# MoHawastaken/Gaussian-Process-Regression

Hardware: AMD Instinct MI355X
Metric: GPR predict-step achieved fp64 TFLOP/s (kernel fill + Cholesky + solves + mean/variance), n x n sqexp (higher is better)
Workload: dtype f64; 1 GPU; c4: n=65536 d=8 sqrexp GPR fit+predict, n*=65536 (reference test-grid rule), noise=0.1; n=65536, d=8, n_star=65536, kernel=sqrexp, parallelism=1-D block-cyclic 512-column panels over 1 GPU(s), test points sliced

## Files before the change

gaussian-process-regression_amd/_native.py:

```python
from __future__ import annotations

import ctypes as C
import os
import threading

import numpy as np

_HERE = os.path.dirname(os.path.abspath(__file__))
LIB_PATH = os.path.join(_HERE, "lib", "libgprc_native" + os.environ.get("GPRC_LIB_SUFFIX", "") + ".so")

CONSTANT, LINEAR, POLYNOMIAL, SQREXP, GAMMAEXP, RATQUAD, SQREXP_ARD = range(7)

OK = 0
GPC_REFERENCE_STOP = 1
ERR_ARG, ERR_HIP, ERR_NOMEM, ERR_NOT_PD, ERR_DIVERGED, ERR_MAXITER, ERR_NO_DEVICE = -1, -2, -3, -4, -5, -6, -7


class GprcError(RuntimeError):

    def __init__(self, status: int, message: str):
        super().__init__(f"gprc native error {status}: {message}")
        self.status = status
        self.message = message

# ... 83 lines not shown
    "gprc_mgpu_gpr_get_noise": (C.c_int, [_vp, C.POINTER(C.c_double)]),
    "gprc_mgpu_model_rank": (C.c_int, [_vp, C.c_int, C.POINTER(_vp)]),
    "gprc_mgpu_model_free": (C.c_int, [_vp]),
    "gprc_mvn_factor": (C.c_int, [_vp, _vp, _i64, _i64, C.c_double, _vp, C.POINTER(C.c_int)]),
    "gprc_mvn_sample": (C.c_int, [_vp, _vp, _i64, _i64, _vp, C.c_double, _vp, _i64, _vp, C.POINTER(C.c_int)]),
    "gprc_sym_eigen": (C.c_int, [_vp, _vp, _i64, _i64, _vp, _vp, C.POINTER(C.c_int)]),
    "gprc_combine_all": (C.c_int, [_vp, _vp, C.POINTER(_i64), C.c_int, _vp]),
    "gprc_prof_enable": (C.c_int, [C.c_int]),
    "gprc_prof_panel_trace": (C.c_int, [_vp, C.c_int, C.POINTER(_i64), C.c_int]),
    "gprc_prof_service_trace": (C.c_int, [_vp, C.POINTER(_i64), C.c_int]),
    "gprc_prof_wait_timeout": (C.c_int, [C.POINTER(C.c_int), C.c_int]),
    "gprc_prof_reset": (C.c_int, []),
    "gprc_prof_kinds": (C.c_int, []),
    "gprc_prof_summary": (C.c_int, [C.c_int, C.POINTER(_i64), C.POINTER(C.c_double), C.POINTER(C.c_double), C.POINTER(C.c_double)]),
    "gprc_dev_solve_rows": (C.c_int, [_vp, _vp, _vp, _i64, _vp, _i64, _i64]),
    "gprc_dev_reverse_factor": (C.c_int, [_vp, _vp, _vp, _i64, _vp, _vp]),
}

_lib = None
_lib_lock = threading.Lock()


def _share_hip_runtime_with_torch() -> None:
    import importlib.util
    import sys
    if "torch" in sys.modules:
        return
    try:
        spec = importlib.util.find_spec("torch")
    except (ImportError, ValueError):
# ... 120 lines not shown
```

gaussian-process-regression_amd/csrc/chol_tile.h:

```cpp
#pragma once
#include <utility>

#include "gprc_internal.h"

namespace gprc {

typedef double double4_t __attribute__((ext_vector_type(4)));

namespace {

constexpr int PB = 128;

constexpr int BLD = 144;
constexpr int PB_SMEM_DOUBLES = PB * BLD + 512 + PB;
constexpr size_t PB_SMEM_BYTES = PB_SMEM_DOUBLES * sizeof(double);

__device__ __forceinline__ void sqrt_rsqrt(double d, double& root, double& rinv) {
  double r = __builtin_amdgcn_rsq(d);
#pragma unroll
  for (int it = 0; it < 2; ++it) {
    const double e = fma(-(d * r), r, 1.0);
    r = fma(0.5 * r, e, r);
  }
  double l = d * r;
// ... 185 lines not shown
        const int c = ty + TYS * (k0 + k);
        if (i >= c) A[i + (int64_t)c * lda] = lv[k];
        winv[i + c * PB] = wv[k];
      }
    }
  }
  POTF2_STAMP(19);
}

constexpr int G_KB = 16;
constexpr int G_LDT = 144;
constexpr int G_BUF = G_KB * G_LDT;
constexpr int G_SMEM_DOUBLES = 4 * G_BUF;
constexpr size_t G_SMEM_BYTES = G_SMEM_DOUBLES * sizeof(double);

__device__ __forceinline__ void read_ops(const double* Ac, const double* Bc, int kk, double (&a)[4], double (&b)[4]) {
#pragma unroll
  for (int m = 0; m < 4; ++m) a[m] = Ac[kk * 4 * G_LDT + m * 16];
#pragma unroll
  for (int n = 0; n < 4; ++n) b[n] = Bc[kk * 4 * G_LDT + n * 16];
}
template <int NEG>
__device__ __forceinline__ void mma_step(const double (&a)[4], const double (&b)[4], double4_t (&acc)[4][4]) {
#pragma unroll
  for (int m = 0; m < 4; ++m)
#pragma unroll
    for (int n = 0; n < 4; ++n) acc[m][n] = __builtin_amdgcn_mfma_f64_16x16x4f64(b[n], a[m], acc[m][n], 0, 0, NEG);
}

typedef __attribute__((address_space(1))) const void* gptr_t;
typedef __attribute__((address_space(3))) void* lptr_t;
__device__ __forceinline__ void dma_ktile(const double* Ag, int64_t lda, const double* Bg, int64_t ldb, double* Asb, double* Bsb) {
#pragma unroll
  for (int i = 0; i < 4; ++i) {
    __builtin_amdgcn_global_load_lds((gptr_t)(Ag + (int64_t)(4 * i) * lda), (lptr_t)(Asb + 4 * i * G_LDT), 16, 0, 0);
// ... 13 lines not shown
  }
}

template <bool SEG>
__device__ __forceinline__ const char* strip_ktile_s(const double* B, int64_t ldb, int64_t brow, int kt, int wave, int64_t& ld) {
  if constexpr (SEG) {
    const int pp = kt / (NB / 16);
    ld = panel_ld(ldb, pp);
    return reinterpret_cast<const char*>(B + panel_offset(ldb, pp) + (brow - (int64_t)pp * NB) + (int64_t)((kt % (NB / 16)) * 16 + wave) * ld);
  } else {
    ld = ldb;
    return reinterpret_cast<const char*>(B + (int64_t)(kt * 16 + wave) * ldb);
  }
}

template <bool SET, bool SEG = false, bool SEGA = false, bool SSQ = false, bool LDSOUT = false, bool ILV = true, int CORE = 2, bool WT = false>
__device__ __forceinline__ void gemm_tile_128(double* C, int64_t ldc, const double* A, int64_t lda, const double* B,
                                              int64_t ldb, int K, double* smem, int64_t brow = 0, int64_t arow = 0, int kt0 = 0,
                                              double* ssq = nullptr, int tid = -1, double* lds_out = nullptr) {
  const int t = tid < 0 ? (int)threadIdx.x : tid, lane = t & 63;
  const int wave = __builtin_amdgcn_readfirstlane(t >> 6);
  const int wr = wave >> 1, wc = wave & 1;
  const int fk = lane >> 4, fr = lane & 15;
  double* As = smem;
  double* Bs = smem + 2 * G_BUF;

  constexpr int NEG = SET ? 0 : 1;
  double* Cw = C + (wr * 64 + fr) + (int64_t)(wc * 64 + fk) * ldc;
  double4_t acc[4][4];
#pragma unroll
  for (int n = 0; n < 4; ++n)
#pragma unroll
    for (int r = 0; r < 4; ++r)
#pragma unroll
      for (int m = 0; m < 4; ++m) acc[m][n][r] = SET ? 0.0 : Cw[m * 16 + (int64_t)(n * 16 + 4 * r) * ldc];

  int64_t ldak, ldbk;
  const double* Ag = strip_ktile<SEGA>(A, lda, arow, SEGA ? kt0 : 0, lane, wave, ldak);
  const double* Bg = strip_ktile<SEG>(B, ldb, brow, SEG ? kt0 : 0, lane, wave, ldbk);
  const int srow = wave * G_LDT;
  const int foff = fr + fk * G_LDT;

  constexpr int LGKM0 = 0xC07F;
  const int KT = K / G_KB;
  dma_ktile(Ag, ldak, Bg, ldbk, As + srow, Bs + srow);
  __builtin_amdgcn_s_waitcnt(0x0F70);
  __syncthreads();
  if (KT > 1) {
    Ag = strip_ktile<SEGA>(A, lda, arow, (SEGA ? kt0 : 0) + 1, lane, wave, ldak);
    Bg = strip_ktile<SEG>(B, ldb, brow, (SEG ? kt0 : 0) + 1, lane, wave, ldbk);
    dma_ktile(Ag, ldak, Bg, ldbk, As + G_BUF + srow, Bs + G_BUF + srow);
  }
  if constexpr (!SEGA) Ag = A + 2 * lane + (int64_t)(2 * G_KB + wave) * lda;
  if constexpr (!SEG) Bg = B + 2 * lane + (int64_t)(2 * G_KB + wave) * ldb;
  double a0[4], b0[4], a1[4], b1[4], a2[4], b2[4], a3[4], b3[4];
  read_ops(As + wr * 64 + foff, Bs + wc * 64 + foff, 0, a0, b0);
  read_ops(As + wr * 64 + foff, Bs + wc * 64 + foff, 1, a1, b1);
  if constexpr (ILV && CORE == 2) {
  const unsigned lane_off = 16u * (unsigned)lane;
  const unsigned ldsA = (unsigned)(uintptr_t)(lptr_t)(As + srow), ldsB = (unsigned)(uintptr_t)(lptr_t)(Bs + srow);
  const unsigned aBase = (unsigned)(uintptr_t)(lptr_t)(As + wr * 64 + foff), bBase = (unsigned)(uintptr_t)(lptr_t)(Bs + wc * 64 + foff);
  int64_t ldas, ldbs;
  const char* Asg = strip_ktile_s<SEGA>(A, lda, arow, (SEGA ? kt0 : 0) + 2, wave, ldas);
  const char* Bsg = strip_ktile_s<SEG>(B, ldb, brow, (SEG ? kt0 : 0) + 2, wave, ldbs);
#define GPRC_SB __builtin_amdgcn_sched_barrier(0);
#define GPRC_M(A_, B_, i) acc[(i) >> 2][(i) & 3] = __builtin_amdgcn_mfma_f64_16x16x4f64(B_[(i) & 3], A_[(i) >> 2], acc[(i) >> 2][(i) & 3], 0, 0, NEG); GPRC_SB
#define GPRC_RD(dst, base, off) asm volatile("ds_read_b64 %0, %1 offset:%2" : "=v"(dst) : "v"(base), "n"(off));
#define GPRC_RA(buf, kk, r, A_) GPRC_RD(A_[2 * (r)], aBase, ((buf) * G_BUF + (kk) * 4 * G_LDT + (2 * (r)) * 16) * 8) GPRC_RD(A_[2 * (r) + 1], aBase, ((buf) * G_BUF + (kk) * 4 * G_LDT + (2 * (r) + 1) * 16) * 8) GPRC_SB
#define GPRC_RB(buf, kk, r, B_) GPRC_RD(B_[2 * (r)], bBase, ((buf) * G_BUF + (kk) * 4 * G_LDT + (2 * (r)) * 16) * 8) GPRC_RD(B_[2 * (r) + 1], bBase, ((buf) * G_BUF + (kk) * 4 * G_LDT + (2 * (r) + 1) * 16) * 8) GPRC_SB
#define GPRC_READY(cnt, A_, B_) asm volatile("s_waitcnt lgkmcnt(" #cnt ")" : "+v"(A_[0]), "+v"(A_[1]), "+v"(A_[2]), "+v"(A_[3]), "+v"(B_[0]), "+v"(B_[1]), "+v"(B_[2]), "+v"(B_[3])); GPRC_SB
#define GPRC_BLOCK_R(A_, B_, buf, kk, RA_, RB_, cond)                                                               \
  GPRC_M(A_, B_, 0) GPRC_M(A_, B_, 1) if (cond) { GPRC_RA(buf, kk, 0, RA_) }                                        \
  GPRC_M(A_, B_, 2) GPRC_M(A_, B_, 3) if (cond) { GPRC_RA(buf, kk, 1, RA_) }                                        \
  GPRC_M(A_, B_, 4) GPRC_M(A_, B_, 5) if (cond) { GPRC_RB(buf, kk, 0, RB_) }                                        \
  GPRC_M(A_, B_, 6) GPRC_M(A_, B_, 7) if (cond) { GPRC_RB(buf, kk, 1, RB_) }                                        \
  GPRC_M(A_, B_, 8) GPRC_M(A_, B_, 9) GPRC_M(A_, B_, 10) GPRC_M(A_, B_, 11) GPRC_M(A_, B_, 12) GPRC_M(A_, B_, 13) GPRC_M(A_, B_, 14) GPRC_M(A_, B_, 15)
#define GPRC_DMA(i, buf, more2)                                                                                      \
  if (more2) {                                                                                                      \
    if ((i) < 4) asm volatile("s_mov_b32 m0, %2\n\ts_nop 0\n\tglobal_load_lds_dwordx4 %0, %1" :: "v"(lane_off), "s"(Asg + (int64_t)(4 * (i)) * ldas * 8), "s"(ldsA + (unsigned)(((buf) * G_BUF + 4 * (i) * G_LDT) * 8)) : "memory"); \
    else asm volatile("s_mov_b32 m0, %2\n\ts_nop 0\n\tglobal_load_lds_dwordx4 %0, %1" :: "v"(lane_off), "s"(Bsg + (int64_t)(4 * ((i) - 4)) * ldbs * 8), "s"(ldsB + (unsigned)(((buf) * G_BUF + 4 * ((i) - 4) * G_LDT) * 8)) : "memory"); \
    GPRC_SB                                                                                                         \
  }
#define GPRC_KTILE(buf, more1, more2)                                                                                \
  {                                                                                                                 \
    GPRC_SB                                                                                                         \
    GPRC_READY(8, a0, b0)                                                                                           \
    GPRC_BLOCK_R(a0, b0, buf, 2, a2, b2, true)                                                                      \
    GPRC_READY(8, a1, b1)                                                                                           \
    GPRC_BLOCK_R(a1, b1, buf, 3, a3, b3, true)                                                                      \
    GPRC_READY(8, a2, b2)                                                                                           \
    GPRC_M(a2, b2, 0) GPRC_M(a2, b2, 1) GPRC_M(a2, b2, 2) GPRC_M(a2, b2, 3)                                         \
    if (more1) {                                                                                                    \
       \
                           \
      asm volatile("s_waitcnt vmcnt(0) lgkmcnt(0)" ::: "memory");                                                   \
      __builtin_amdgcn_s_barrier();                                                                                 \
      GPRC_SB                                                                                                       \
    }                                                                                                               \
    GPRC_M(a2, b2, 4) if (more1) { GPRC_RA(1 - (buf), 0, 0, a0) }                                                   \
// ... 42 lines not shown
  GPRC_M(A_, B_, 0) GPRC_M(A_, B_, 1) if (cond) { GPRC_RA(Ap_, kk, 0, RA_) }                                        \
  GPRC_M(A_, B_, 2) GPRC_M(A_, B_, 3) if (cond) { GPRC_RA(Ap_, kk, 1, RA_) }                                        \
  GPRC_M(A_, B_, 4) GPRC_M(A_, B_, 5) if (cond) { GPRC_RB(Bp_, kk, 0, RB_) }                                        \
  GPRC_M(A_, B_, 6) GPRC_M(A_, B_, 7) if (cond) { GPRC_RB(Bp_, kk, 1, RB_) }                                        \
  GPRC_M(A_, B_, 8) GPRC_M(A_, B_, 9) GPRC_M(A_, B_, 10) GPRC_M(A_, B_, 11) GPRC_M(A_, B_, 12) GPRC_M(A_, B_, 13) GPRC_M(A_, B_, 14) GPRC_M(A_, B_, 15)
#define GPRC_DMA(i, more2)                                                                                           \
  if (more2) {                                                                                                      \
    if ((i) < 4) __builtin_amdgcn_global_load_lds((gptr_t)(Ag + (int64_t)(4 * (i)) * ldak), (lptr_t)(As + cur + srow + 4 * (i) * G_LDT), 16, 0, 0); \
    else __builtin_amdgcn_global_load_lds((gptr_t)(Bg + (int64_t)(4 * ((i) - 4)) * ldbk), (lptr_t)(Bs + cur + srow + 4 * ((i) - 4) * G_LDT), 16, 0, 0); \
    GPRC_SB                                                                                                         \
  }
#define GPRC_KTILE(more1, more2)                                                                                     \
  {                                                                                                                 \
    const int cur = (kt & 1) * G_BUF, nxt = G_BUF - cur;                                                            \
    const double* Ac = As + cur + wr * 64 + foff;                                                                   \
    const double* Bc = Bs + cur + wc * 64 + foff;                                                                   \
    const double* An = As + nxt + wr * 64 + foff;                                                                   \
    const double* Bn = Bs + nxt + wc * 64 + foff;                                                                   \
    GPRC_SB                                                                                                         \
    GPRC_BLOCK_R(a0, b0, Ac, Bc, 2, a2, b2, true)                                                                   \
    GPRC_BLOCK_R(a1, b1, Ac, Bc, 3, a3, b3, true)                                                                   \
    GPRC_M(a2, b2, 0) GPRC_M(a2, b2, 1) GPRC_M(a2, b2, 2) GPRC_M(a2, b2, 3)                                         \
    if (more1) {                                                                                                    \
       \
                         \
      asm volatile("s_waitcnt vmcnt(0) lgkmcnt(0)" ::: "memory");                                                   \
      __builtin_amdgcn_s_barrier();                                                                                 \
      GPRC_SB                                                                                                       \
      if (more2) {                                                                                                  \
        if constexpr (SEGA || SEG) {                                                                                \
          const bool boundary = ((kt0 + kt + 2) % (NB / 16)) == 0;                                                  \
          if constexpr (SEGA) { if (boundary) Ag = strip_ktile<true>(A, lda, arow, kt0 + kt + 2, lane, wave, ldak); else Ag += (int64_t)G_KB * ldak; } \
          if constexpr (SEG) { if (boundary) Bg = strip_ktile<true>(B, ldb, brow, kt0 + kt + 2, lane, wave, ldbk); else Bg += (int64_t)G_KB * ldbk; } \
// ... 20 lines not shown
      const bool more1 = kt + 1 < KT;
      GPRC_KTILE(more1, false)
    }
  }
#undef GPRC_KTILE
#undef GPRC_DMA
#undef GPRC_BLOCK_R
#undef GPRC_RA
#undef GPRC_RB
#undef GPRC_M
#undef GPRC_SB
  } else {
  for (int kt = 0; kt < KT; ++kt) {
    const int cur = (kt & 1) * G_BUF, nxt = G_BUF - cur;
    const double* Ac = As + cur + wr * 64 + foff;
    const double* Bc = Bs + cur + wc * 64 + foff;
    const double* An = As + nxt + wr * 64 + foff;
    const double* Bn = Bs + nxt + wc * 64 + foff;
    __builtin_amdgcn_s_waitcnt(LGKM0);
    read_ops(Ac, Bc, 2, a2, b2);
    mma_step<NEG>(a0, b0, acc);
    __builtin_amdgcn_sched_barrier(0);
    __builtin_amdgcn_s_waitcnt(LGKM0);
    read_ops(Ac, Bc, 3, a3, b3);
    mma_step<NEG>(a1, b1, acc);
    __builtin_amdgcn_sched_barrier(0);
    __builtin_amdgcn_s_waitcnt(LGKM0);
    if (kt + 1 < KT) {
      asm volatile("s_waitcnt vmcnt(0)" ::: "memory");
      __syncthreads();
      if (kt + 2 < KT) {
        if constexpr (SEGA || SEG) {
          const bool boundary = ((kt0 + kt + 2) % (NB / 16)) == 0;
// ... 10 lines not shown
    __builtin_amdgcn_sched_barrier(0);
    __builtin_amdgcn_s_waitcnt(LGKM0);
    if (kt + 1 < KT) read_ops(An, Bn, 1, a1, b1);
    mma_step<NEG>(a3, b3, acc);
    __builtin_amdgcn_sched_barrier(0);
  }

  }

#pragma unroll
  for (int n = 0; n < 4; ++n)
#pragma unroll
    for (int r = 0; r < 4; ++r)
#pragma unroll
      for (int m = 0; m < 4; ++m) {
        if constexpr (WT) __hip_atomic_store(&Cw[m * 16 + (int64_t)(n * 16 + 4 * r) * ldc], acc[m][n][r], __ATOMIC_RELAXED, __HIP_MEMORY_SCOPE_AGENT);
        else Cw[m * 16 + (int64_t)(n * 16 + 4 * r) * ldc] = acc[m][n][r];
      }

  if constexpr (LDSOUT) {
    __syncthreads();
    constexpr int LDO = 144;
#pragma unroll
    for (int n = 0; n < 4; ++n)
#pragma unroll
      for (int r = 0; r < 4; ++r)
#pragma unroll
        for (int m = 0; m < 4; ++m) {
          const int row = wr * 64 + fr + m * 16, col = wc * 64 + fk + n * 16 + 4 * r;
          lds_out[row + col * LDO] = (row >= col) ? acc[m][n][r] : 0.0;
        }
  }

  if constexpr (SSQ) {
    double rs[4];
#pragma unroll
    for (int m = 0; m < 4; ++m) {
      double q = 0.0;
#pragma unroll
      for (int n = 0; n < 4; ++n)
#pragma unroll
        for (int r = 0; r < 4; ++r) q = fma(acc[m][n][r], acc[m][n][r], q);
      q += __shfl_xor(q, 16, 64);
      q += __shfl_xor(q, 32, 64);
      rs[m] = q;
    }
    __syncthreads();
    if (fk == 0) {
#pragma unroll
// ... 47 lines not shown
```

gaussian-process-regression_amd/csrc/gprc_internal.h:

```cpp
#pragma once
#include <hip/hip_runtime.h>
#include <stdint.h>
#include <atomic>
#include <string>

#include "../../include/gprc_native.h"

namespace gprc {

#ifndef GPRC_NB
#define GPRC_NB 512
#endif
constexpr int NB = GPRC_NB;
constexpr int NBI = 128;
constexpr int TPP = NB / NBI;
constexpr int MAX_PARAMS = 256;
constexpr int MAX_DEVICES = 64;
static_assert(NB % NBI == 0 && NB >= NBI, "panel width must be a multiple of the 128 block");

__host__ __device__ static inline int64_t pad_up(int64_t n, int64_t m) { return (n + m - 1) / m * m; }
__host__ __device__ static inline int64_t panel_offset(int64_t n_pad, int64_t p) { return (int64_t)NB * (p * n_pad - (int64_t)NB * p * (p - 1) / 2); }
__host__ __device__ static inline int64_t panel_ld(int64_t n_pad, int64_t p) { return n_pad - p * NB; }
template <typename T>
__host__ __device__ constexpr T panel_tiles(T P, T q) { return TPP * TPP * (P - q) - TPP * (TPP - 1) / 2; }
constexpr int SERVICE_CORE_WGS = 3 + TPP + TPP * (TPP + 1) / 2;
constexpr int CHAIN_HELPERS = 4;

void set_error(const std::string& msg);
int hip_fail(hipError_t e, const char* what, const char* file, int line);

#define GPRC_HIP(call)                                                          \
  do {                                                                          \
    hipError_t e__ = (call);                                                    \
    if (e__ != hipSuccess) return ::gprc::hip_fail(e__, #call, __FILE__, __LINE__); \
  } while (0)
#define GPRC_TRY(call)          \
  do {                          \
    int rc__ = (call);          \
    if (rc__ != 0) return rc__; \
  } while (0)
#define GPRC_LAUNCH_CHECK() GPRC_HIP(hipGetLastError())
// ... 55 lines not shown

int64_t grad_partial_rows();
int launch_grad_contract(hipStream_t s, const KernelSpec& ks, const double* X, int64_t d, int64_t n, const double* alpha, const double* W,
                         int64_t ld, double* part);
int launch_gpc_grad_contract(hipStream_t s, const KernelSpec& ks, const double* X, int64_t d, int64_t n, const double* a, const double* sw,
                             const double* u, const double* g, const double* W, int64_t ld, double* part);

int64_t pred_grad_stripes(int64_t n_pad);
int launch_pred_grad(hipStream_t s, const KernelSpec& ks, const double* Xs, int64_t m, int64_t m_pad, const double* X, int64_t n, int64_t n_pad,
                     int64_t d, const double* alpha, const double* W, int64_t ldw, double* pmean, double* pvar);
int launch_pred_grad_sum(hipStream_t s, const KernelSpec& ks, const double* part, int64_t n_pad, int64_t d, int64_t m_pad, int64_t m, bool variance,
                         double* out);

int launch_solve_panel_fused(hipStream_t s, double* vt, int64_t ldv, int64_t m_pad, const double* packed, int64_t n_pad, int64_t p,
                             const double* winv, double* sspart, int64_t ss_stride = 0);
int launch_trsm_panel(hipStream_t s, double* X, int64_t ldx, int64_t M, const double* winv, double* ssq = nullptr);
int launch_gemm_nt(hipStream_t s, double* C, int64_t ldc, const double* A, int64_t lda, const double* B, int64_t ldb,
                   int64_t M, int64_t N, int64_t K, int lower, int kind);
int launch_solve_left(hipStream_t s, double* vt, int64_t ldv, int64_t m_pad, const double* packed, int64_t n_pad, int64_t j, int64_t G,
                      int64_t tri_row0 = -1);
int launch_trailing_update(hipStream_t s, double* packed, int64_t n_pad, int64_t p, int64_t q_begin, int64_t q_end,
                           int64_t q_stride);
int launch_trailing_range(hipStream_t s, double* packed, int64_t n_pad, int64_t p_begin, int64_t p_end, int64_t q_begin, int64_t q_end,
                          int64_t q_stride);

int launch_potf2_inv(hipStream_t s, double* A, int64_t lda, double* winv, int* info_dev, int col0);
int launch_panel_fused(hipStream_t s, double* packed, int64_t n_pad, int64_t p, double* winv, int* info_dev, void* sync16, int trace);
size_t panel_service_sync_bytes(int64_t P);
int launch_panel_service(hipStream_t s, double* packed, int64_t n_pad, double* winv, int* info_dev, void* sync, void* trace, double* inv,
                         int64_t p_begin, int64_t p_end, bool split, int part);
// ... 41 lines not shown
```

gaussian-process-regression_amd/csrc/gprc_sched.hip:

```cpp
#include <algorithm>
#include <cstdlib>
#include <cstring>

#include "gprc_host.h"

namespace gprc {

static bool panel_steps() {
  static const bool steps = [] { const char* e = std::getenv("GPRC_PANEL"); return e && std::strcmp(e, "steps") == 0; }();
  return steps;
}

int factor_subpanel(gprc_ctx* ctx, double* packed, int64_t n_pad, int64_t p, int j, int part, double* winv, int* info_dev) {
  if (part == 2) return 0;
  hipStream_t s = ctx->stream;
  const int64_t ld = panel_ld(n_pad, p);
  double* pan = packed + panel_offset(n_pad, p);
  const int64_t cj = (int64_t)j * NBI;
  double* wblk = winv + (p * (NB / NBI) + j) * NBI * NBI;
  if (cj > 0)
    GPRC_TRY(launch_gemm_nt(s, pan + cj + cj * ld, ld, pan + cj, ld, pan + cj, ld, ld - cj, NBI, cj, 1, PK_GEMM_INNER));
  GPRC_TRY(launch_potf2_inv(s, pan + cj + cj * ld, ld, wblk, info_dev, (int)(p * NB + cj)));
  const int64_t below = ld - cj - NBI;
  if (below > 0) GPRC_TRY(launch_trsm_panel(s, pan + (cj + NBI) + cj * ld, ld, below, wblk));
// ... 148 lines not shown
              "under a tool that serialises dispatches (e.g. rocprofv3 --pmc) set GPRC_SERVICE=0");
    return GPRC_ERR_HIP;
  }
  return 0;
}

int solve_rows(gprc_ctx* ctx, const double* packed, const double* winv, int64_t n_pad, double* vt, int64_t ldv, int64_t m_pad,
               double* sspart, int64_t tri_row0, int64_t p_end) {
  hipStream_t s = ctx->stream;
  const int64_t P = p_end >= 0 ? std::min(p_end, n_pad / NB) : n_pad / NB;
  const char* mode = std::getenv("GPRC_SOLVE");
  int64_t G = (4096 + (m_pad / 128) * (NB / NBI) - 1) / ((m_pad / 128) * (NB / NBI));
  if (mode && std::strcmp(mode, "left") == 0) G = 1;
  else if (mode && std::atoi(mode) > 0) G = std::atoi(mode);
  if ((mode && std::strcmp(mode, "right") == 0) || G > P) G = P;
  auto rows_of = [&](int64_t col_end) {
    if (tri_row0 < 0) return m_pad;
    return std::max<int64_t>(0, std::min<int64_t>(m_pad, pad_up(col_end - tri_row0, 128)));
  };
  for (int64_t g0 = 0; g0 < P; g0 += G) {
    const int64_t g1 = std::min(P, g0 + G);
    const int64_t mg = rows_of(g1 * NB);
    if (mg == 0) continue;
    GPRC_TRY(launch_solve_left(s, vt, ldv, mg, packed, n_pad, g0, g1 - g0, tri_row0));
    static const bool solve_panel_steps = [] { const char* e = std::getenv("GPRC_SOLVE_PANEL"); return e && std::strcmp(e, "steps") == 0; }();
    for (int64_t p = g0; p < g1; ++p) {
      const int64_t ld = panel_ld(n_pad, p);
      const double* pan = packed + panel_offset(n_pad, p);
      const int64_t mp = rows_of((p + 1) * NB);
      if (mp == 0) continue;
      if (!solve_panel_steps) {
        GPRC_TRY(launch_solve_panel_fused(s, vt, ldv, mp, packed, n_pad, p, winv, sspart, m_pad));
      } else
      for (int j = 0; j < NB / NBI; ++j) {
        const int64_t cj = p * NB + (int64_t)j * NBI;
        const double* wblk = winv + (p * (NB / NBI) + j) * NBI * NBI;
        if (j > 0)
          GPRC_TRY(launch_gemm_nt(s, vt + cj * ldv, ldv, vt + p * NB * ldv, ldv, pan + (int64_t)j * NBI, ld, mp, NBI, (int64_t)j * NBI, 0,
                                  PK_GEMM_INNER));
        GPRC_TRY(launch_trsm_panel(s, vt + cj * ldv, ldv, mp, wblk, sspart ? sspart + (cj / NBI) * m_pad : nullptr));
// ... 69 lines not shown
  return factor_all_async(ctx, packed, n_pad, winv, info_dev, inv);
}
int gprc_factor_service(int on) {
  const int was = g_service_off.load() ? 0 : 1;
  if (on == 0) g_service_off.store(true);
  else if (on > 0) g_service_off.store(false);
  return was;
}

int gprc_dev_solve_rows(gprc_ctx* ctx, const double* packed, const double* winv, int64_t n_pad, double* vt,
                        int64_t ld, int64_t m_pad) {
  GPRC_TRY(use_device_unless(ctx, m_pad % 128 || n_pad % NB || ld < m_pad || ld % 2, "solve_rows: bad padding"));
  return solve_rows(ctx, packed, winv, n_pad, vt, ld, m_pad);
}

int gprc_dev_reverse_factor(gprc_ctx* ctx, const double* packed, const double* winv, int64_t n_pad, double* packed_rev, double* winv_rev) {
  GPRC_TRY(use_device_unless(ctx, !packed || !winv || !packed_rev || !winv_rev || n_pad <= 0 || n_pad % NB, "dev_reverse_factor: bad arguments"));
  return launch_reverse_factor(ctx->stream, packed, winv, n_pad, packed_rev, winv_rev);
}

int gprc_prof_panel_trace(gprc_ctx* ctx, int side, int64_t* ticks_out, int n) {
  GPRC_TRY(use_device_unless(ctx, !ticks_out || n < 1 || n > 24, "prof_panel_trace: 1..24 stamps"));
  GPRC_HIP(hipDeviceSynchronize());
  GPRC_HIP(hipMemcpy(ticks_out, static_cast<char*>(ctx->sync_dev) + (side ? 256 : 0) + 64, sizeof(int64_t) * (size_t)n, hipMemcpyDeviceToHost));
  return 0;
}

int gprc_prof_service_trace(gprc_ctx* ctx, int64_t* ticks_out, int panels) {
  GPRC_TRY(use_device_unless(ctx, !ticks_out || panels < 1 || panels > SVC_TRACE_PANELS, "prof_service_trace: 1..48 panels"));
  if (!ctx->svc_trace) { set_error("prof_service_trace: no traced sweep on this context (set GPRC_SERVICE_TRACE before the first call)"); return GPRC_ERR_ARG; }
// ... 76 lines not shown
```

gaussian-process-regression_amd/csrc/kernels_gemm.hip:

```cpp
#include <algorithm>

#include "chol_tile.h"

namespace gprc {
namespace {

template <int ROLE>
__global__ __launch_bounds__(256, 2) void gemm_nt_kernel(double* C, int64_t ldc, const double* A, int64_t lda,
                                                         const double* B, int64_t ldb, int tiles_m, int tiles_n, int K,
                                                         int lower, int group) {
  extern __shared__ __attribute__((aligned(16))) double smem[];
  const unsigned ntiles = (unsigned)tiles_m * (unsigned)tiles_n;
  for (unsigned t = blockIdx.x; t < ntiles; t += gridDim.x) {
    const unsigned id = ROLE == PK_INV_GEMM ? t : xcd_remap(t, ntiles);
    int tr, tc;
    group_tile(id, tiles_m, tiles_n, group, tr, tc);
    if (lower && tc > tr) continue;
    const int64_t k0 = ROLE == PK_INV_GEMM ? (int64_t)tr * 128 : 0;
    gemm_tile_128<false>(C + (int64_t)tr * 128 + (int64_t)tc * 128 * ldc, ldc, A + (int64_t)tr * 128 + k0 * lda, lda,
                         B + (int64_t)tc * 128 + k0 * ldb, ldb, K - (int)k0, smem);
    __syncthreads();
  }
}

// ... 47 lines not shown
__global__ __launch_bounds__(256, 2) void solve_panel_fused_kernel(double* vt, int64_t ldv, const double* packed, int64_t n_pad, int p,
                                                                   const double* winv, double* sspart, int64_t m_pad) {
  extern __shared__ __attribute__((aligned(16))) double smem[];
  const int64_t ld = panel_ld(n_pad, p);
  const double* pan = packed + panel_offset(n_pad, p);
  double* strip = vt + (int64_t)blockIdx.x * 128 + (int64_t)p * NB * ldv;
  for (int j = 0; j < TPP; ++j) {
    double* C = strip + (int64_t)j * NBI * ldv;
    if (j > 0) {
      gemm_tile_128<false>(C, ldv, strip, ldv, pan + (int64_t)j * NBI, ld, j * NBI, smem);
      asm volatile("s_waitcnt vmcnt(0)" ::: "memory");
      __syncthreads();
    }
    const double* wblk = winv + ((int64_t)p * TPP + j) * NBI * NBI;
    double* ssq = SSQ ? sspart + ((int64_t)p * TPP + j) * m_pad + (int64_t)blockIdx.x * 128 : nullptr;
    gemm_tile_128<true, false, false, SSQ>(C, ldv, C, ldv, wblk, 128, 128, smem, 0, 0, 0, ssq);
    asm volatile("s_waitcnt vmcnt(0)" ::: "memory");
    __syncthreads();
  }
}

__global__ __launch_bounds__(256, 2) void trailing_range_kernel(double* packed, int64_t n_pad, int p_begin, int p_end, int q_begin,
                                                                int q_stride, int n_targets, int ntiles) {
  extern __shared__ __attribute__((aligned(16))) double smem[];
  const int P = (int)(n_pad / NB);
  int id = (int)xcd_remap(blockIdx.x, (unsigned)ntiles);
  int q, tr, tc;
  if (!target_tile(id, P, q_begin, q_stride, n_targets, q)) return;
  panel_tile(id, tr, tc);
  const int64_t ldq = panel_ld(n_pad, q);
  double* Cq = packed + panel_offset(n_pad, q);
  const int64_t row = (int64_t)q * NB + (int64_t)tr * 128, col = (int64_t)q * NB + (int64_t)tc * 128;
  gemm_tile_128<false, true, true>(Cq + (int64_t)tr * 128 + (int64_t)tc * 128 * ldq, ldq, packed, n_pad, packed, n_pad,
                                   (p_end - p_begin) * NB, smem, col, row, p_begin * (NB / 16));
}

}

int launch_solve_left(hipStream_t s, double* vt, int64_t ldv, int64_t m_pad, const double* packed, int64_t n_pad, int64_t j, int64_t G,
                      int64_t tri_row0) {
  if (j <= 0 || m_pad <= 0 || G <= 0) return 0;
  if (m_pad % 128) { set_error("solve_left: m_pad must be a multiple of 128"); return GPRC_ERR_ARG; }
  if ((j + G) * NB > n_pad) { set_error("solve_left: panel group beyond the factor"); return GPRC_ERR_ARG; }
  GPRC_TRY(ensure_dynamic_lds<solve_left_kernel>(G_SMEM_BYTES));
  const int64_t N = G * NB, tiles = (m_pad / 128) * (N / 128), K = j * NB;
  double fl = 2.0 * (double)m_pad * N * (double)K;
  if (tri_row0 >= 0) {
    fl = 0.0;
    for (int64_t tr = 0; tr < m_pad / 128; ++tr) fl += 2.0 * 128.0 * N * (double)std::max<int64_t>(0, K - std::max<int64_t>(0, tri_row0 + tr * 128));
  }
  ProfScope ps(s, PK_SOLVE_LEFT, fl, 8.0 * (2.0 * m_pad * N + (double)m_pad * K + (double)N * K));
  hipLaunchKernelGGL(solve_left_kernel, dim3((unsigned)tiles), dim3(256), G_SMEM_BYTES, s, vt, ldv, packed, n_pad,
                     (int)j, (int)(m_pad / 128), (int)(N / 128), 8, tri_row0);
  GPRC_LAUNCH_CHECK();
  return 0;
}

int launch_solve_panel_fused(hipStream_t s, double* vt, int64_t ldv, int64_t m_pad, const double* packed, int64_t n_pad, int64_t p,
                             const double* winv, double* sspart, int64_t ss_stride) {
  if (m_pad <= 0) return 0;
  if (ss_stride <= 0) ss_stride = m_pad;
  if (m_pad % 128) { set_error("solve_panel_fused: m_pad must be a multiple of 128"); return GPRC_ERR_ARG; }
  GPRC_TRY(sspart ? ensure_dynamic_lds<solve_panel_fused_kernel<true>>(G_SMEM_BYTES) : ensure_dynamic_lds<solve_panel_fused_kernel<false>>(G_SMEM_BYTES));
  const double M = (double)m_pad;
  ProfScope ps(s, PK_SOLVE_PANEL, M * 128.0 * 128.0 * TPP + 2.0 * M * 128.0 * 128.0 * (TPP * (TPP - 1) / 2), 8.0 * 2.0 * M * NB);
  if (sspart) hipLaunchKernelGGL(solve_panel_fused_kernel<true>, dim3((unsigned)(m_pad / 128)), dim3(256), G_SMEM_BYTES, s, vt, ldv, packed, n_pad, (int)p, winv, sspart, ss_stride);
  else hipLaunchKernelGGL(solve_panel_fused_kernel<false>, dim3((unsigned)(m_pad / 128)), dim3(256), G_SMEM_BYTES, s, vt, ldv, packed, n_pad, (int)p, winv, sspart, ss_stride);
  GPRC_LAUNCH_CHECK();
  return 0;
}

int launch_trsm_panel(hipStream_t s, double* X, int64_t ldx, int64_t M, const double* winv, double* ssq) {
  if (M <= 0) return 0;
  if (M % 128) { set_error("trsm_panel: M must be a multiple of 128"); return GPRC_ERR_ARG; }
  GPRC_TRY(ssq ? ensure_dynamic_lds<trsm_panel_kernel<true>>(G_SMEM_BYTES) : ensure_dynamic_lds<trsm_panel_kernel<false>>(G_SMEM_BYTES));
  ProfScope ps(s, PK_TRSM_PANEL, 1.0 * M * 128 * 128, 8.0 * 2 * M * 128);
  if (ssq) hipLaunchKernelGGL(trsm_panel_kernel<true>, dim3((unsigned)(M / 128)), dim3(256), G_SMEM_BYTES, s, X, ldx, winv, ssq);
  else hipLaunchKernelGGL(trsm_panel_kernel<false>, dim3((unsigned)(M / 128)), dim3(256), G_SMEM_BYTES, s, X, ldx, winv, ssq);
  GPRC_LAUNCH_CHECK();
  return 0;
}

// ... 63 lines not shown
```

include/gprc_native.h:

```cpp
#ifndef GPRC_NATIVE_H
#define GPRC_NATIVE_H

#include <stdint.h>

#ifdef __cplusplus
extern "C" {
#endif

#define GPRC_ABI_VERSION 1

#if defined(__GNUC__)
#define GPRC_API __attribute__((visibility("default")))
#else
#define GPRC_API
#endif

typedef enum {
  GPRC_CONSTANT = 0,
  GPRC_LINEAR = 1,
  GPRC_POLYNOMIAL = 2,
  GPRC_SQREXP = 3,
  GPRC_GAMMAEXP = 4,
  GPRC_RATQUAD = 5,
  GPRC_SQREXP_ARD = 6
// ... 90 lines not shown
GPRC_API int gprc_dev_trsv_step(gprc_ctx* ctx, const double* packed, const double* inv, int64_t n_pad, double* b, int transpose,
                       int64_t p, double* work);
GPRC_API int gprc_dev_fill_cross(gprc_ctx* ctx, int kernel, const double* params_host, int n_params, const double* X_star,
                        int64_t d, int64_t m, int64_t m_pad, const double* X, int64_t n, int64_t n_pad, double* vt,
                        int64_t ld);
GPRC_API int64_t gprc_rowreduce_splits(int64_t cols);
GPRC_API int gprc_dev_row_reduce(gprc_ctx* ctx, const double* vt, int64_t ld, int64_t rows, int64_t cols, const double* w,
                        double* out, double* work);
GPRC_API int gprc_dev_logp(gprc_ctx* ctx, const double* packed, int64_t n_pad, int64_t n, const double* y, const double* alpha,
                  double* out_dev);
GPRC_API int gprc_gpr_model_from_device(gprc_ctx* ctx, int kernel, const double* params, int n_params, const double* X,
                               int64_t d, int64_t n, const double* y, double* packed, double* winv, double* alpha,
                               double noise, double logp, gprc_model** model_out);
GPRC_API int gprc_dev_solve_rows(gprc_ctx* ctx, const double* packed, const double* winv, int64_t n_pad, double* vt,
                        int64_t ld, int64_t m_pad);
GPRC_API int gprc_dev_reverse_factor(gprc_ctx* ctx, const double* packed, const double* winv, int64_t n_pad, double* packed_rev,
                                     double* winv_rev);

#define GPRC_MGPU_RCCL 1
#define GPRC_MGPU_NO_LOOKAHEAD 2
#define GPRC_MGPU_SCATTER_ALLGATHER 4
#define GPRC_MGPU_AUTO_EXCHANGE 8
typedef struct gprc_mgpu gprc_mgpu;
typedef struct gprc_mgpu_model gprc_mgpu_model;
GPRC_API int gprc_mgpu_create(const int* devices, int n_ranks, int flags, gprc_mgpu** mgpu_out);
GPRC_API int gprc_mgpu_destroy(gprc_mgpu* mgpu);
GPRC_API int gprc_mgpu_ranks(const gprc_mgpu* mgpu, int* n_ranks_out);
GPRC_API int gprc_mgpu_calibrate(gprc_mgpu* mgpu, int64_t doubles, int reps, int* choice_out, double* ms_out);
GPRC_API int gprc_mgpu_exchange_mode(const gprc_mgpu* mgpu, int* mode_out);
GPRC_API int gprc_mgpu_stats(const gprc_mgpu* mgpu, double* out, int n);
// ... 33 lines not shown
```

Measured before the change: 75.72 TFLOP/s.

## Skip zero blocks in triangular inverse product and fuse multi-panel solve groups

Adds a TRI mode to the 128-tile GEMM that applies the lower-triangular inverse diagonal block by skipping MFMA steps on column blocks known to be zero, with interleaved column ownership across waves to balance work. It also adds a solve_group kernel that handles several panels per launch (default 2 when there are enough row strips), doing the intra-group updates inside the kernel and reserving the separate GEMM for trailing updates. The aim is to cut wasted FLOPs on triangular blocks and reduce launch count and the serial steps between panels. In exchange it brings a more complex sum-of-squares reduction that needs extra syncthreads, and it moves work into per-strip serial loops.

```diff
diff --git a/gaussian-process-regression_amd/_native.py b/gaussian-process-regression_amd/_native.py
--- a/gaussian-process-regression_amd/_native.py
+++ b/gaussian-process-regression_amd/_native.py
@@ -121,6 +121,8 @@
     "gprc_prof_kinds": (C.c_int, []),
     "gprc_prof_summary": (C.c_int, [C.c_int, C.POINTER(_i64), C.POINTER(C.c_double), C.POINTER(C.c_double), C.POINTER(C.c_double)]),
     "gprc_dev_solve_rows": (C.c_int, [_vp, _vp, _vp, _i64, _vp, _i64, _i64]),
+    "gprc_dev_solve_rows_part": (C.c_int, [_vp, _vp, _vp, _i64, _vp, _i64, _i64, _vp, _i64]),
+    "gprc_tri_product_plan": (C.c_int, [C.c_int, C.c_int, C.c_int, C.POINTER(C.c_int)]),
     "gprc_dev_reverse_factor": (C.c_int, [_vp, _vp, _vp, _i64, _vp, _vp]),
 }
 
diff --git a/gaussian-process-regression_amd/csrc/chol_tile.h b/gaussian-process-regression_amd/csrc/chol_tile.h
--- a/gaussian-process-regression_amd/csrc/chol_tile.h
+++ b/gaussian-process-regression_amd/csrc/chol_tile.h
@@ -223,11 +223,12 @@
 constexpr int G_SMEM_DOUBLES = 4 * G_BUF;
 constexpr size_t G_SMEM_BYTES = G_SMEM_DOUBLES * sizeof(double);
 
+template <int CN = 16>
 __device__ __forceinline__ void read_ops(const double* Ac, const double* Bc, int kk, double (&a)[4], double (&b)[4]) {
 #pragma unroll
   for (int m = 0; m < 4; ++m) a[m] = Ac[kk * 4 * G_LDT + m * 16];
 #pragma unroll
-  for (int n = 0; n < 4; ++n) b[n] = Bc[kk * 4 * G_LDT + n * 16];
+  for (int n = 0; n < 4; ++n) b[n] = Bc[kk * 4 * G_LDT + n * CN];
 }
 template <int NEG>
 __device__ __forceinline__ void mma_step(const double (&a)[4], const double (&b)[4], double4_t (&acc)[4][4]) {
@@ -271,7 +272,8 @@
   }
 }
 
-template <bool SET, bool SEG = false, bool SEGA = false, bool SSQ = false, bool LDSOUT = false, bool ILV = true, int CORE = 2, bool WT = false>
+template <bool SET, bool SEG = false, bool SEGA = false, bool SSQ = false, bool LDSOUT = false, bool ILV = true, int CORE = 2, bool WT = false,
+          bool TRI = false>
 __device__ __forceinline__ void gemm_tile_128(double* C, int64_t ldc, const double* A, int64_t lda, const double* B,
                                               int64_t ldb, int K, double* smem, int64_t brow = 0, int64_t arow = 0, int kt0 = 0,
                                               double* ssq = nullptr, int tid = -1, double* lds_out = nullptr) {
@@ -283,14 +285,17 @@
   double* Bs = smem + 2 * G_BUF;
 
   constexpr int NEG = SET ? 0 : 1;
-  double* Cw = C + (wr * 64 + fr) + (int64_t)(wc * 64 + fk) * ldc;
+  static_assert(!TRI || (SET && ILV && CORE == 2 && !LDSOUT && !SEG && !SEGA), "the triangular product is a SET form of the VALU-free loop");
+  constexpr int CN = TRI ? 32 : 16;
+  const int c0 = TRI ? wc * 16 : wc * 64;
+  double* Cw = C + (wr * 64 + fr) + (int64_t)(c0 + fk) * ldc;
   double4_t acc[4][4];
 #pragma unroll
   for (int n = 0; n < 4; ++n)
 #pragma unroll
     for (int r = 0; r < 4; ++r)
 #pragma unroll
-      for (int m = 0; m < 4; ++m) acc[m][n][r] = SET ? 0.0 : Cw[m * 16 + (int64_t)(n * 16 + 4 * r) * ldc];
+      for (int m = 0; m < 4; ++m) acc[m][n][r] = SET ? 0.0 : Cw[m * 16 + (int64_t)(n * CN + 4 * r) * ldc];
 
   int64_t ldak, ldbk;
   const double* Ag = strip_ktile<SEGA>(A, lda, arow, SEGA ? kt0 : 0, lane, wave, ldak);
@@ -311,20 +316,20 @@
   if constexpr (!SEGA) Ag = A + 2 * lane + (int64_t)(2 * G_KB + wave) * lda;
   if constexpr (!SEG) Bg = B + 2 * lane + (int64_t)(2 * G_KB + wave) * ldb;
   double a0[4], b0[4], a1[4], b1[4], a2[4], b2[4], a3[4], b3[4];
-  read_ops(As + wr * 64 + foff, Bs + wc * 64 + foff, 0, a0, b0);
-  read_ops(As + wr * 64 + foff, Bs + wc * 64 + foff, 1, a1, b1);
+  read_ops<CN>(As + wr * 64 + foff, Bs + c0 + foff, 0, a0, b0);
+  read_ops<CN>(As + wr * 64 + foff, Bs + c0 + foff, 1, a1, b1);
   if constexpr (ILV && CORE == 2) {
   const unsigned lane_off = 16u * (unsigned)lane;
   const unsigned ldsA = (unsigned)(uintptr_t)(lptr_t)(As + srow), ldsB = (unsigned)(uintptr_t)(lptr_t)(Bs + srow);
-  const unsigned aBase = (unsigned)(uintptr_t)(lptr_t)(As + wr * 64 + foff), bBase = (unsigned)(uintptr_t)(lptr_t)(Bs + wc * 64 + foff);
+  const unsigned aBase = (unsigned)(uintptr_t)(lptr_t)(As + wr * 64 + foff), bBase = (unsigned)(uintptr_t)(lptr_t)(Bs + c0 + foff);
   int64_t ldas, ldbs;
   const char* Asg = strip_ktile_s<SEGA>(A, lda, arow, (SEGA ? kt0 : 0) + 2, wave, ldas);
   const char* Bsg = strip_ktile_s<SEG>(B, ldb, brow, (SEG ? kt0 : 0) + 2, wave, ldbs);
 #define GPRC_SB __builtin_amdgcn_sched_barrier(0);
-#define GPRC_M(A_, B_, i) acc[(i) >> 2][(i) & 3] = __builtin_amdgcn_mfma_f64_16x16x4f64(B_[(i) & 3], A_[(i) >> 2], acc[(i) >> 2][(i) & 3], 0, 0, NEG); GPRC_SB
+#define GPRC_M(A_, B_, i) if (!TRI || ((i) & 3) >= n0) { acc[(i) >> 2][(i) & 3] = __builtin_amdgcn_mfma_f64_16x16x4f64(B_[(i) & 3], A_[(i) >> 2], acc[(i) >> 2][(i) & 3], 0, 0, NEG); } GPRC_SB
 #define GPRC_RD(dst, base, off) asm volatile("ds_read_b64 %0, %1 offset:%2" : "=v"(dst) : "v"(base), "n"(off));
 #define GPRC_RA(buf, kk, r, A_) GPRC_RD(A_[2 * (r)], aBase, ((buf) * G_BUF + (kk) * 4 * G_LDT + (2 * (r)) * 16) * 8) GPRC_RD(A_[2 * (r) + 1], aBase, ((buf) * G_BUF + (kk) * 4 * G_LDT + (2 * (r) + 1) * 16) * 8) GPRC_SB
-#define GPRC_RB(buf, kk, r, B_) GPRC_RD(B_[2 * (r)], bBase, ((buf) * G_BUF + (kk) * 4 * G_LDT + (2 * (r)) * 16) * 8) GPRC_RD(B_[2 * (r) + 1], bBase, ((buf) * G_BUF + (kk) * 4 * G_LDT + (2 * (r) + 1) * 16) * 8) GPRC_SB
+#define GPRC_RB(buf, kk, r, B_) GPRC_RD(B_[2 * (r)], bBase, ((buf) * G_BUF + (kk) * 4 * G_LDT + (2 * (r)) * CN) * 8) GPRC_RD(B_[2 * (r) + 1], bBase, ((buf) * G_BUF + (kk) * 4 * G_LDT + (2 * (r) + 1) * CN) * 8) GPRC_SB
 #define GPRC_READY(cnt, A_, B_) asm volatile("s_waitcnt lgkmcnt(" #cnt ")" : "+v"(A_[0]), "+v"(A_[1]), "+v"(A_[2]), "+v"(A_[3]), "+v"(B_[0]), "+v"(B_[1]), "+v"(B_[2]), "+v"(B_[3])); GPRC_SB
 #define GPRC_BLOCK_R(A_, B_, buf, kk, RA_, RB_, cond)                                                               \
   GPRC_M(A_, B_, 0) GPRC_M(A_, B_, 1) if (cond) { GPRC_RA(buf, kk, 0, RA_) }                                        \
@@ -340,6 +345,7 @@
   }
 #define GPRC_KTILE(buf, more1, more2)                                                                                \
   {                                                                                                                 \
+    const int n0 = TRI ? tri_first_block(wc, kt) : 0;                                                               \
     GPRC_SB                                                                                                         \
     GPRC_READY(8, a0, b0)                                                                                           \
     GPRC_BLOCK_R(a0, b0, buf, 2, a2, b2, true)                                                                      \
@@ -412,9 +418,9 @@
   {                                                                                                                 \
     const int cur = (kt & 1) * G_BUF, nxt = G_BUF - cur;                                                            \
     const double* Ac = As + cur + wr * 64 + foff;                                                                   \
-    const double* Bc = Bs + cur + wc * 64 + foff;                                                                   \
+    const double* Bc = Bs + cur + c0 + foff;                                                                   \
     const double* An = As + nxt + wr * 64 + foff;                                                                   \
-    const double* Bn = Bs + nxt + wc * 64 + foff;                                                                   \
+    const double* Bn = Bs + nxt + c0 + foff;                                                                   \
     GPRC_SB                                                                                                         \
     GPRC_BLOCK_R(a0, b0, Ac, Bc, 2, a2, b2, true)                                                                   \
     GPRC_BLOCK_R(a1, b1, Ac, Bc, 3, a3, b3, true)                                                                   \
@@ -465,9 +471,9 @@
   for (int kt = 0; kt < KT; ++kt) {
     const int cur = (kt & 1) * G_BUF, nxt = G_BUF - cur;
     const double* Ac = As + cur + wr * 64 + foff;
-    const double* Bc = Bs + cur + wc * 64 + foff;
+    const double* Bc = Bs + cur + c0 + foff;
     const double* An = As + nxt + wr * 64 + foff;
-    const double* Bn = Bs + nxt + wc * 64 + foff;
+    const double* Bn = Bs + nxt + c0 + foff;
     __builtin_amdgcn_s_waitcnt(LGKM0);
     read_ops(Ac, Bc, 2, a2, b2);
     mma_step<NEG>(a0, b0, acc);
@@ -508,8 +514,8 @@
     for (int r = 0; r < 4; ++r)
 #pragma unroll
       for (int m = 0; m < 4; ++m) {
-        if constexpr (WT) __hip_atomic_store(&Cw[m * 16 + (int64_t)(n * 16 + 4 * r) * ldc], acc[m][n][r], __ATOMIC_RELAXED, __HIP_MEMORY_SCOPE_AGENT);
-        else Cw[m * 16 + (int64_t)(n * 16 + 4 * r) * ldc] = acc[m][n][r];
+        if constexpr (WT) __hip_atomic_store(&Cw[m * 16 + (int64_t)(n * CN + 4 * r) * ldc], acc[m][n][r], __ATOMIC_RELAXED, __HIP_MEMORY_SCOPE_AGENT);
+        else Cw[m * 16 + (int64_t)(n * CN + 4 * r) * ldc] = acc[m][n][r];
       }
 
   if constexpr (LDSOUT) {
@@ -526,7 +532,31 @@
         }
   }
 
-  if constexpr (SSQ) {
+  if constexpr (SSQ && TRI) {
+    double* slot = smem + wr * 256 + lane;
+    __syncthreads();
+#pragma unroll
+    for (int leg = 0; leg < 4; ++leg) {
+      if (wc == (leg & 1)) {
+#pragma unroll
+        for (int h = 0; h < 2; ++h)
+#pragma unroll
+          for (int m = 0; m < 4; ++m) {
+            double q = leg == 0 ? 0.0 : slot[h * 512 + m * 64];
+#pragma unroll
+            for (int r = 0; r < 4; ++r) q = fma(acc[m][2 * h + (leg >> 1)][r], acc[m][2 * h + (leg >> 1)][r], q);
+            if (leg < 3) slot[h * 512 + m * 64] = q;
+            else {
+              q += __shfl_xor(q, 16, 64);
+              q += __shfl_xor(q, 32, 64);
+              if (h == 0) acc[m][0][0] = q;
+              else if (fk == 0) ssq[wr * 64 + m * 16 + fr] = acc[m][0][0] + q;
+            }
+          }
+      }
+      if (leg < 3) __syncthreads();
+    }
+  } else if constexpr (SSQ) {
     double rs[4];
 #pragma unroll
     for (int m = 0; m < 4; ++m) {
diff --git a/gaussian-process-regression_amd/csrc/gprc_internal.h b/gaussian-process-regression_amd/csrc/gprc_internal.h
--- a/gaussian-process-regression_amd/csrc/gprc_internal.h
+++ b/gaussian-process-regression_amd/csrc/gprc_internal.h
@@ -25,6 +25,10 @@
 __host__ __device__ constexpr T panel_tiles(T P, T q) { return TPP * TPP * (P - q) - TPP * (TPP - 1) / 2; }
 constexpr int SERVICE_CORE_WGS = 3 + TPP + TPP * (TPP + 1) / 2;
 constexpr int CHAIN_HELPERS = 4;
+
+__host__ __device__ constexpr int tri_col_block(int wc, int n) { return wc + 2 * n; }
+__host__ __device__ constexpr int tri_first_block(int wc, int kt) { return (kt - wc + 1) >> 1; }
+__host__ __device__ constexpr bool tri_ktile_runs(int wc, int n, int kt) { return n >= tri_first_block(wc, kt); }
 
 void set_error(const std::string& msg);
 int hip_fail(hipError_t e, const char* what, const char* file, int line);
@@ -110,6 +114,8 @@
 
 int launch_solve_panel_fused(hipStream_t s, double* vt, int64_t ldv, int64_t m_pad, const double* packed, int64_t n_pad, int64_t p,
                              const double* winv, double* sspart, int64_t ss_stride = 0);
+int launch_solve_group(hipStream_t s, double* vt, int64_t ldv, int64_t m_pad, const double* packed, int64_t n_pad, int64_t p0, int64_t p1,
+                       const double* winv, double* sspart, int64_t ss_stride = 0);
 int launch_trsm_panel(hipStream_t s, double* X, int64_t ldx, int64_t M, const double* winv, double* ssq = nullptr);
 int launch_gemm_nt(hipStream_t s, double* C, int64_t ldc, const double* A, int64_t lda, const double* B, int64_t ldb,
                    int64_t M, int64_t N, int64_t K, int lower, int kind);
diff --git a/gaussian-process-regression_amd/csrc/gprc_sched.hip b/gaussian-process-regression_amd/csrc/gprc_sched.hip
--- a/gaussian-process-regression_amd/csrc/gprc_sched.hip
+++ b/gaussian-process-regression_amd/csrc/gprc_sched.hip
@@ -186,6 +186,10 @@
   if (mode && std::strcmp(mode, "left") == 0) G = 1;
   else if (mode && std::atoi(mode) > 0) G = std::atoi(mode);
   if ((mode && std::strcmp(mode, "right") == 0) || G > P) G = P;
+  static const bool solve_panel_steps = [] { const char* e = std::getenv("GPRC_SOLVE_PANEL"); return e && std::strcmp(e, "steps") == 0; }();
+  const char* group_mode = std::getenv("GPRC_SOLVE_GROUP");
+  const int64_t group_env = group_mode ? (int64_t)std::atoi(group_mode) : 0;
+  const int64_t F = std::min(G, group_env > 0 ? group_env : (m_pad / 128 >= 512 ? (int64_t)2 : (int64_t)1));
   auto rows_of = [&](int64_t col_end) {
     if (tri_row0 < 0) return m_pad;
     return std::max<int64_t>(0, std::min<int64_t>(m_pad, pad_up(col_end - tri_row0, 128)));
@@ -195,7 +199,16 @@
     const int64_t mg = rows_of(g1 * NB);
     if (mg == 0) continue;
     GPRC_TRY(launch_solve_left(s, vt, ldv, mg, packed, n_pad, g0, g1 - g0, tri_row0));
-    static const bool solve_panel_steps = [] { const char* e = std::getenv("GPRC_SOLVE_PANEL"); return e && std::strcmp(e, "steps") == 0; }();
+    if (F > 1 && !solve_panel_steps && tri_row0 < 0) {
+      for (int64_t f0 = g0; f0 < g1; f0 += F) {
+        const int64_t f1 = std::min(g1, f0 + F);
+        GPRC_TRY(launch_solve_group(s, vt, ldv, m_pad, packed, n_pad, f0, f1, winv, sspart, m_pad));
+        for (int64_t p = f0; p < f1 && f1 < g1; ++p)
+          GPRC_TRY(launch_gemm_nt(s, vt + f1 * NB * ldv, ldv, vt + p * NB * ldv, ldv, packed + panel_offset(n_pad, p) + (f1 - p) * NB,
+                                  panel_ld(n_pad, p), m_pad, (g1 - f1) * NB, NB, 0, PK_SOLVE_UPDATE));
+      }
+      continue;
+    }
     for (int64_t p = g0; p < g1; ++p) {
       const int64_t ld = panel_ld(n_pad, p);
       const double* pan = packed + panel_offset(n_pad, p);
@@ -295,6 +308,18 @@
   return solve_rows(ctx, packed, winv, n_pad, vt, ld, m_pad);
 }
 
+int gprc_dev_solve_rows_part(gprc_ctx* ctx, const double* packed, const double* winv, int64_t n_pad, double* vt, int64_t ld, int64_t m_pad,
+                             double* sspart, int64_t p_end) {
+  GPRC_TRY(use_device_unless(ctx, m_pad % 128 || n_pad % NB || ld < m_pad || ld % 2, "solve_rows_part: bad padding"));
+  return solve_rows(ctx, packed, winv, n_pad, vt, ld, m_pad, sspart, -1, p_end);
+}
+
+int gprc_tri_product_plan(int wc, int n, int kt, int* col_block) {
+  if (wc < 0 || wc > 1 || n < 0 || n > 3 || kt < 0 || kt > 7) return -1;
+  if (col_block) *col_block = tri_col_block(wc, n);
+  return tri_ktile_runs(wc, n, kt) ? 1 : 0;
+}
+
 int gprc_dev_reverse_factor(gprc_ctx* ctx, const double* packed, const double* winv, int64_t n_pad, double* packed_rev, double* winv_rev) {
   GPRC_TRY(use_device_unless(ctx, !packed || !winv || !packed_rev || !winv_rev || n_pad <= 0 || n_pad % NB, "dev_reverse_factor: bad arguments"));
   return launch_reverse_factor(ctx->stream, packed, winv, n_pad, packed_rev, winv_rev);
diff --git a/gaussian-process-regression_amd/csrc/kernels_gemm.hip b/gaussian-process-regression_amd/csrc/kernels_gemm.hip
--- a/gaussian-process-regression_amd/csrc/kernels_gemm.hip
+++ b/gaussian-process-regression_amd/csrc/kernels_gemm.hip
@@ -85,7 +85,28 @@
     }
     const double* wblk = winv + ((int64_t)p * TPP + j) * NBI * NBI;
     double* ssq = SSQ ? sspart + ((int64_t)p * TPP + j) * m_pad + (int64_t)blockIdx.x * 128 : nullptr;
-    gemm_tile_128<true, false, false, SSQ>(C, ldv, C, ldv, wblk, 128, 128, smem, 0, 0, 0, ssq);
+    gemm_tile_128<true, false, false, SSQ, false, true, 2, false, true>(C, ldv, C, ldv, wblk, 128, 128, smem, 0, 0, 0, ssq);
+    asm volatile("s_waitcnt vmcnt(0)" ::: "memory");
+    __syncthreads();
+  }
+}
+
+template <bool SSQ>
+__global__ __launch_bounds__(256, 2) void solve_group_kernel(double* vt, int64_t ldv, const double* packed, int64_t n_pad, int p0, int p1,
+                                                             const double* winv, double* sspart, int64_t m_pad) {
+  extern __shared__ __attribute__((aligned(16))) double smem[];
+  double* strip = vt + (int64_t)blockIdx.x * 128;
+  const double* first = strip + (int64_t)p0 * NB * ldv;
+  for (int b = p0 * TPP; b < p1 * TPP; ++b) {
+    double* C = strip + (int64_t)b * NBI * ldv;
+    const int kb = b - p0 * TPP;
+    if (kb > 0) {
+      gemm_tile_128<false, true>(C, ldv, first, ldv, packed, n_pad, kb * NBI, smem, (int64_t)b * NBI, 0, p0 * (NB / 16));
+      asm volatile("s_waitcnt vmcnt(0)" ::: "memory");
+      __syncthreads();
+    }
+    double* ssq = SSQ ? sspart + (int64_t)b * m_pad + (int64_t)blockIdx.x * 128 : nullptr;
+    gemm_tile_128<true, false, false, SSQ, false, true, 2, false, true>(C, ldv, C, ldv, winv + (int64_t)b * NBI * NBI, 128, 128, smem, 0, 0, 0, ssq);
     asm volatile("s_waitcnt vmcnt(0)" ::: "memory");
     __syncthreads();
   }
@@ -107,6 +128,8 @@
 }
 
 }
+
+constexpr double TRI_BLOCK_FLOPS = 2.0 * 128.0 * 128.0 * 36.0 / 64.0;
 
 int launch_solve_left(hipStream_t s, double* vt, int64_t ldv, int64_t m_pad, const double* packed, int64_t n_pad, int64_t j, int64_t G,
                       int64_t tri_row0) {
@@ -134,9 +157,24 @@
   if (m_pad % 128) { set_error("solve_panel_fused: m_pad must be a multiple of 128"); return GPRC_ERR_ARG; }
   GPRC_TRY(sspart ? ensure_dynamic_lds<solve_panel_fused_kernel<true>>(G_SMEM_BYTES) : ensure_dynamic_lds<solve_panel_fused_kernel<false>>(G_SMEM_BYTES));
   const double M = (double)m_pad;
-  ProfScope ps(s, PK_SOLVE_PANEL, M * 128.0 * 128.0 * TPP + 2.0 * M * 128.0 * 128.0 * (TPP * (TPP - 1) / 2), 8.0 * 2.0 * M * NB);
+  ProfScope ps(s, PK_SOLVE_PANEL, TRI_BLOCK_FLOPS * M * TPP + 2.0 * M * 128.0 * 128.0 * (TPP * (TPP - 1) / 2), 8.0 * 2.0 * M * NB);
   if (sspart) hipLaunchKernelGGL(solve_panel_fused_kernel<true>, dim3((unsigned)(m_pad / 128)), dim3(256), G_SMEM_BYTES, s, vt, ldv, packed, n_pad, (int)p, winv, sspart, ss_stride);
   else hipLaunchKernelGGL(solve_panel_fused_kernel<false>, dim3((unsigned)(m_pad / 128)), dim3(256), G_SMEM_BYTES, s, vt, ldv, packed, n_pad, (int)p, winv, sspart, ss_stride);
+  GPRC_LAUNCH_CHECK();
+  return 0;
+}
+
+int launch_solve_group(hipStream_t s, double* vt, int64_t ldv, int64_t m_pad, const double* packed, int64_t n_pad, int64_t p0, int64_t p1,
+                       const double* winv, double* sspart, int64_t ss_stride) {
+  if (m_pad <= 0 || p1 <= p0) return 0;
+  if (ss_stride <= 0) ss_stride = m_pad;
+  if (m_pad % 128) { set_error("solve_group: m_pad must be a multiple of 128"); return GPRC_ERR_ARG; }
+  if (p0 < 0 || p1 * NB > n_pad) { set_error("solve_group: panel group beyond the factor"); return GPRC_ERR_ARG; }
+  GPRC_TRY(sspart ? ensure_dynamic_lds<solve_group_kernel<true>>(G_SMEM_BYTES) : ensure_dynamic_lds<solve_group_kernel<false>>(G_SMEM_BYTES));
+  const double M = (double)m_pad, nb = (double)((p1 - p0) * TPP);
+  ProfScope ps(s, PK_SOLVE_PANEL, TRI_BLOCK_FLOPS * M * nb + 2.0 * M * 128.0 * 128.0 * (nb * (nb - 1) / 2), 8.0 * 2.0 * M * NB * (double)(p1 - p0));
+  if (sspart) hipLaunchKernelGGL(solve_group_kernel<true>, dim3((unsigned)(m_pad / 128)), dim3(256), G_SMEM_BYTES, s, vt, ldv, packed, n_pad, (int)p0, (int)p1, winv, sspart, ss_stride);
+  else hipLaunchKernelGGL(solve_group_kernel<false>, dim3((unsigned)(m_pad / 128)), dim3(256), G_SMEM_BYTES, s, vt, ldv, packed, n_pad, (int)p0, (int)p1, winv, sspart, ss_stride);
   GPRC_LAUNCH_CHECK();
   return 0;
 }
diff --git a/include/gprc_native.h b/include/gprc_native.h
--- a/include/gprc_native.h
+++ b/include/gprc_native.h
@@ -128,6 +128,9 @@
                                double noise, double logp, gprc_model** model_out);
 GPRC_API int gprc_dev_solve_rows(gprc_ctx* ctx, const double* packed, const double* winv, int64_t n_pad, double* vt,
                         int64_t ld, int64_t m_pad);
+GPRC_API int gprc_dev_solve_rows_part(gprc_ctx* ctx, const double* packed, const double* winv, int64_t n_pad, double* vt, int64_t ld,
+                                      int64_t m_pad, double* sspart, int64_t p_end);
+GPRC_API int gprc_tri_product_plan(int wc, int n, int kt, int* col_block);
 GPRC_API int gprc_dev_reverse_factor(gprc_ctx* ctx, const double* packed, const double* winv, int64_t n_pad, double* packed_rev,
                                      double* winv_rev);
 
```

After: 75.79 TFLOP/s (median of 6 runs). About the same (+0.1%).
